# python-microscopy/ch-shrinkwrap

Measured on AMD Instinct MI355X. Metric: vertex-updates/s (force+CG step) + achieved HBM GB/s, 1M pts/200k verts, higher is better.
Workload: dtype f32; 1 GPU; BASELINE configs[2]: two-lobe vesicle (smooth union of two R=300 nm spheres), 1000000 localizations sigma=10 nm, 198812 vertices / 397620 faces, lams=[10], blocks of 5 iterations, fixed topology; localizations_per_gpu=1000000, vertices_per_gpu=198812, faces_per_gpu=397620, block=5, mode=single, parallelism=single GPU

## Files before the change

ch_shrinkwrap_amd/build.py:

```python
import glob
import os
import subprocess

HERE = os.path.dirname(os.path.abspath(__file__))
LIB = os.path.join(HERE, 'libnanowrap_hip.so')


def _csrc(name):
    return os.path.join(HERE, 'csrc', name)


def _include(name):
    return os.path.join(os.path.dirname(HERE), 'include', name)


HIPCC_FLAGS = ['-O3', '--offload-arch=gfx950', '-fPIC', '-shared', '-ffp-contract=off', '-munsafe-fp-atomics',
               '-fvisibility=hidden', '-Wall', '-Wno-unused-function']
_BASE = ['-O3', '--offload-arch=gfx950', '-fPIC', '-fvisibility=hidden']
_QUERY = _BASE + ['-ffp-contract=off', '-Wall', '-Wno-unused-function']
_BQ_H = [_csrc('nw_bq.h'), _csrc('nw_bq_core.h')]
_BQ = _BQ_H + [_csrc('nw_device.h')]

OBJ_MAIN, OBJ_HOLEPUNCH, OBJ_SURGERY, OBJ_BQ = _csrc('nanowrap.o'), _csrc('nw_holepunch.o'), _csrc('nw_surgery.o'), _csrc('nw_bq.o')
OBJ_ISOSURFACE = _csrc('nw_isosurface.o')
# ... 50 lines not shown
        if verbose:
            print(' '.join(cmd))
        subprocess.check_call(cmd)

    for src, obj, extra, flags in UNITS:
        if force or not os.path.exists(obj) or os.path.getmtime(obj) < max(os.path.getmtime(d) for d in [src] + extra):
            run([hipcc] + flags + ['-c', '-o', obj, src])
    check_kernel_budgets(verbose=verbose)
    run([hipcc, '--offload-arch=gfx950', '-fPIC', '-shared', '-o', LIB] + [obj for _, obj, _, _ in UNITS])
    return LIB


LLVM_BIN = os.environ.get('NW_LLVM_BIN', '/opt/rocm/lib/llvm/bin')
KERNEL_BUDGETS = {
    'k_nn_wave<false>':               (80, 10 * 1024),
    'k_attract':                      (72, 20 * 1024),
    'k_face_centroids':               (64, 8 * 1024),
    'k_centroid_scatter':             (64, 0),
    'k_scan_final':                   (64, 1024),
    'k_prior_ring':                   (128, 1024),
    'k_prior_directions':             (96, 1024),
    'k_subspace_point_sums':          (128, 1024),
    'k_solve_update':                 (128, 1024),
    'k_hp_empty_faces':               (64, 0),
    'k_hp_pair':                      (64, 8 * 1024),
    'k_hp_prism':                     (176, 0),
    'k_hp_cand_geom':                 (32, 0),
    'k_hp_pair_final':                (16, 0),
    'k_ws_init':                      (16, 0),
    'k_ws_hook':                      (32, 0),
    'k_ws_compress':                  (16, 0),
    'k_ws_number':                    (16, 0),
    'k_ws_stats':                     (64, 0),
    'k_ws_bbox_init':                 (16, 0),
    'k_ws_active':                    (16, 0),
    'k_ws_winding':                   (176, 0),
    'k_ws_lengths':                   (16, 0),
    'k_ws_hist':                      (16, 2048),
    'k_ws_pick':                      (32, 0),
    'k_ws_flag':                      (16, 0),
    'k_iso_count':                    (16, 16 * 1024),
    'k_iso_widen':                    (16, 0),
    'k_iso_smooth':                   (16, 0),
    'k_iso_hist':                     (16, 1024),
    'k_iso_pattern':                  (32, 0),
    'k_iso_compact':                  (16, 0),
# ... 152 lines not shown
```

ch_shrinkwrap_amd/csrc/nanowrap.hip:

```cpp
#include <hip/hip_runtime.h>
#include <cstdio>
#include <cstdlib>
#include <cstring>
#include <cmath>
#include <string>
#include <vector>
#include <algorithm>
#include <chrono>
#include <thread>
#include <atomic>

#include "../../include/nanowrap.h"
#include "nw_kernels.h"
#include "nw_host_copy.h"

int nw_sort_pairs_u32(const unsigned *key_in, unsigned *key_out, const int *val_in, int *val_out, int n, int bits, hipStream_t stream);

static_assert(sizeof(NwIterLogDev) == sizeof(nw_iter_log), "device/host log record mismatch");
static_assert(SC_COUNT <= NW_N_SCALARS, "scalar slots");

#define NW_EXPORT extern "C" __attribute__((visibility("default")))

#include <dlfcn.h>
#include <rccl/rccl.h>
struct NwRccl {
    void *lib = nullptr;
    ncclResult_t (*GetUniqueId)(ncclUniqueId *) = nullptr;
    ncclResult_t (*CommInitRank)(ncclComm_t *, int, ncclUniqueId, int) = nullptr;
    ncclResult_t (*CommDestroy)(ncclComm_t) = nullptr;
    ncclResult_t (*AllReduce)(const void *, void *, size_t, ncclDataType_t, ncclRedOp_t, ncclComm_t, hipStream_t) = nullptr;
    ncclResult_t (*Send)(const void *, size_t, ncclDataType_t, int, ncclComm_t, hipStream_t) = nullptr;
    ncclResult_t (*Recv)(void *, size_t, ncclDataType_t, int, ncclComm_t, hipStream_t) = nullptr;
    ncclResult_t (*GroupStart)() = nullptr;
    ncclResult_t (*GroupEnd)() = nullptr;
    const char *(*GetErrorString)(ncclResult_t) = nullptr;
    std::string err;
// ... 99 lines not shown
    double cell_tune = 1.0;
    bool tuned = false;
    int blocks_done = 0;
    double force_h = 0.0;
    DevBuf<int> ccount, cstart, scan_tmp;
    DevBuf<int> ctile;
    DevBuf<float> data_in, dat;
    bool have_data = false;
    DevBuf<NwItem> items;
    DevBuf<unsigned> item_cost;
    bool handoff_off = false;
    DevBuf<int> query_serial;
    DevBuf<int> item_done;
    bool items_by_cost = false;
    bool item_cost_valid = false;
    int nitems = 0;
    int item_level = -1;
    DevBuf<int> aux_i;
    DevBuf<float> aux_f, aux_f2, aux_f3;
    DevBuf<double> aux_d;
    DevBuf<unsigned long long> nn_stats;
    DevBuf<unsigned> proj_key;
    DevBuf<int> proj_idx;
    bool proj_ready = false, proj_sorted = false;
    bool face_warm = false;

    DevBuf<float> pos, meshpos, nrm;
    DevBuf<int> nbr, nbr_t, faces;
    DevBuf<unsigned char> valid, owned;
    bool have_valid = false, have_owned = false;
    DevBuf<int> hb_local, hb_slot, hb_slot2local, hb_gv;
    DevBuf<long long> halo_acc;
    DevBuf<float> halo_rows;
    DevBuf<float> halo_full;
    DevBuf<float> halo_ref;
    DevBuf<float> halo_d0;
    bool have_halo_d0 = false;
    int64_t halo_d0_n = 0;
    DevBuf<float> halo_stats;
    void *pin_full = nullptr;
    size_t pin_full_bytes = 0;
    bool full_staged = false;
    bool have_halo_ref = false;
    int64_t hb_n = 0, hb_nslot = 0, M_global = 0;
    bool have_boundary = false;
    bool pos_unpack_pending = false;
    bool have_peers = false;
// ... 146 lines not shown
    const double sr = ctx->sigma_eff > 0 ? std::min(std::max(ctx->sigma_eff / sp, 1.0), 16.0) : 4.0;
    double h = 2.9 * sp * std::pow(sr, 0.3) * std::pow(ratio, -0.11);
    const char *e = getenv("NW_CELL_FACTOR");
    if (e && atof(e) > 0) h *= atof(e);
    return std::max(h, 0.5 * mean_dist) * ctx->cell_tune;
}

int ensure_item_done(nw_ctx *ctx)
{
    const size_t want = (size_t)std::max(ctx->nitems, 1) + 256;
    if (!ctx->query_serial.p) {
        NW_HIP(ctx->query_serial.ensure(1));
        NW_HIP(hipMemsetAsync(ctx->query_serial.p, 0, sizeof(int), ctx->stream));
    }
    if (ctx->item_done.n < want) {
        NW_HIP(ctx->item_done.ensure(2 * want));
        NW_HIP(hipMemsetAsync(ctx->item_done.p, 0, 2 * want * sizeof(int), ctx->stream));
    }
    const size_t rows = (size_t)(ctx->nitems + 8 * 16 + 8);
    if (ctx->part_a.n < 5 * rows) NW_HIP(ctx->part_a.ensure(5 * rows));
    return NW_OK;
}

int build_items(nw_ctx *ctx, int level)
{
    const int64_t N = ctx->N;
    int ipts = (N >= 64 * 9216) ? NW_ITEM_POINTS : NW_ITEM_POINTS / 2;
    if (const char *e = getenv("NW_ITEM_PTS")) ipts = std::max(8, std::min(NW_ITEM_POINTS, atoi(e)));
    if (level == ctx->item_level && ctx->nitems > 0 && ipts == ctx->item_points) return NW_OK;
    ctx->item_points = ipts;
    DevBuf<int> head, hscan, bstart, icount, istart;
    NW_HIP(head.ensure(N)); NW_HIP(hscan.ensure(N + 1));
    hipLaunchKernelGGL(k_block_heads, dim3(nblk(N)), dim3(NW_BLOCK), 0, ctx->stream, ctx->mkey.p, (int)N, 3 * level, head.p);
    NW_TRY(scan_exclusive(ctx, head.p, (int)N, hscan.p));
    int nblocks = 0;
    NW_HIP(hipMemcpyAsync(&nblocks, hscan.p + N, sizeof(int), hipMemcpyDeviceToHost, ctx->stream));
    NW_HIP(hipStreamSynchronize(ctx->stream));
    NW_HIP(bstart.ensure((size_t)nblocks + 1)); NW_HIP(icount.ensure((size_t)nblocks)); NW_HIP(istart.ensure((size_t)nblocks + 1));
    hipLaunchKernelGGL(k_block_starts, dim3(nblk(N)), dim3(NW_BLOCK), 0, ctx->stream, head.p, hscan.p, (int)N, bstart.p);
    hipLaunchKernelGGL(k_block_item_counts, dim3(nblk(nblocks)), dim3(NW_BLOCK), 0, ctx->stream, bstart.p, nblocks, icount.p, ctx->item_points);
    NW_TRY(scan_exclusive(ctx, icount.p, nblocks, istart.p));
    int nitems = 0;
    NW_HIP(hipMemcpyAsync(&nitems, istart.p + nblocks, sizeof(int), hipMemcpyDeviceToHost, ctx->stream));
    NW_HIP(hipStreamSynchronize(ctx->stream));
    NW_HIP(ctx->items.ensure((size_t)nitems));
    hipLaunchKernelGGL(k_block_fill_items, dim3(nblk(nblocks)), dim3(NW_BLOCK), 0, ctx->stream, bstart.p, istart.p, nblocks, ctx->items.p, ctx->item_points);
    NW_HIP(hipGetLastError());
    NW_HIP(hipStreamSynchronize(ctx->stream));
    ctx->nitems = nitems;
    ctx->item_level = level;
    NW_HIP(ctx->item_cost.ensure((size_t)2 * nitems));
    NW_HIP(hipMemsetAsync(ctx->item_cost.p, 0, (size_t)2 * nitems * sizeof(unsigned), ctx->stream));
    NW_TRY(ensure_item_done(ctx));
    ctx->items_by_cost = false; ctx->item_cost_valid = false;
    if (getenv("NW_VERBOSE"))
        fprintf(stderr, "[nanowrap] work list: Morton level %d (block %.2f), %d blocks, %d items (%.1f localizations per wave)\n", level,
                ctx->morton_unit * (float)(1 << level), nblocks, nitems, (double)N / std::max(nitems, 1));
    return NW_OK;
}

int build_grid(nw_ctx *ctx, double mean_dist)
{
    const int64_t N = ctx->N, F = ctx->F;
    float mlo[3], mhi[3];
    bool bad = false;
    NW_TRY(minmax3(ctx, ctx->meshpos.p, ctx->M, mlo, mhi, &bad));
    if (bad) return fail(ctx, NW_ERR_NONFINITE, "non-finite vertex coordinate");
    NW_HIP(ctx->wsum.ensure(4));
    NW_HIP(hipMemsetAsync(ctx->wsum.p + 1, 0, 2 * sizeof(double), ctx->stream));
    hipLaunchKernelGGL(k_mesh_area, dim3(std::min(1024, nblk(F))), dim3(NW_BLOCK), 0, ctx->stream, ctx->meshpos.p, ctx->faces.p, (int)F, ctx->wsum.p + 1);
    const int nsample = (int)std::min<int64_t>(N, 256);
    if (mean_dist <= 0.0)
        hipLaunchKernelGGL(k_sample_nn, dim3(nsample), dim3(NW_BLOCK), 0, ctx->stream, ctx->pts_in.p, N, nsample, ctx->meshpos.p, ctx->faces.p, (int)F, ctx->wsum.p + 2);
    NW_HIP(hipGetLastError());
    double h2[2];
    NW_HIP(hipMemcpyAsync(h2, ctx->wsum.p + 1, sizeof(h2), hipMemcpyDeviceToHost, ctx->stream));
    NW_HIP(hipStreamSynchronize(ctx->stream));
// ... 316 lines not shown
                           1.0f / ctx->morton_unit, key_in.p, idx_in.p);
        NW_HIP(hipGetLastError());
        const int se = nw_sort_pairs_u32(key_in.p, ctx->mkey.p, idx_in.p, ctx->perm.p, (int)N, 30, ctx->stream);
        if (se != 0) return fail(ctx, NW_ERR_HIP, std::string("radix sort of the Morton keys: ") + hipGetErrorString((hipError_t)se));
        NW_HIP(ctx->pts.ensure(N));
        NW_HIP(ctx->mask.ensure(N));
        if (ctx->sinv_array) NW_HIP(ctx->sinv.ensure(3 * N));
        if (ctx->w_array) NW_HIP(ctx->wnorm.ensure(3 * N));
        const float *w_src = ctx->w_array ? ((ctx->w_mode == NW_WEIGHTS_ARRAY || ctx->w_mode == NW_WEIGHTS_PRENORMALIZED) ? ctx->w_in.p : ctx->sinv_in.p) : nullptr;
        hipLaunchKernelGGL(k_point_gather, dim3(nblk(N)), dim3(NW_BLOCK), 0, ctx->stream, (int)N, ctx->pts_in.p, ctx->perm.p,
                           ctx->sinv_array ? ctx->sinv_in.p : nullptr, w_src, ctx->wsum.p, ctx->w_array ? (ctx->w_mode == NW_WEIGHTS_PRENORMALIZED ? 2 : 1) : 0,
                           ctx->pts.p, ctx->sinv_array ? ctx->sinv.p : nullptr, ctx->w_array ? ctx->wnorm.p : nullptr, ctx->mask.p);
        NW_HIP(hipGetLastError());
        NW_HIP(hipStreamSynchronize(ctx->stream));
    }
    ctx->have_points = true;
    ctx->have_data = false;
    ctx->grid_valid = false;
    ctx->item_level = -1;
    ctx->nitems = 0;
    ctx->face_warm = false;
    if (verbose_level() >= 2) fprintf(stderr, "[nanowrap] warm start dropped (%s)\n", __func__);
    ctx->proj_ready = false; ctx->proj_sorted = false;
    ctx->tuned = false; ctx->cell_tune = 1.0; ctx->blocks_done = 0;
    ctx->last_mean_dist = -1.0;
    ctx->searched = false;
    return NW_OK;
}

static int gather_data(nw_ctx *ctx)
{
    const int64_t N = ctx->N;
    if (ctx->have_data) NW_HIP(ctx->dat.ensure(3 * N));
    hipLaunchKernelGGL(k_data_gather, dim3(nblk(N)), dim3(NW_BLOCK), 0, ctx->stream, (int)N, ctx->perm.p, ctx->have_data ? ctx->data_in.p : nullptr, ctx->pts.p,
                       ctx->have_data ? ctx->dat.p : nullptr, ctx->w_array ? nullptr : ctx->mask.p);
    NW_HIP(hipGetLastError());
    return NW_OK;
}

NW_EXPORT int nw_set_data(nw_ctx *ctx, const float *data)
{
    if (!ctx) return NW_ERR_BADARG;
    if (!ctx->have_points) return fail(ctx, NW_ERR_BADARG, "nw_set_data: set the localizations first");
    if (ctx->in_search) return fail(ctx, NW_ERR_BADARG, "nw_set_data inside a search");
    NW_HIP(hipSetDevice(ctx->device));
    if (!data && !ctx->have_data) return NW_OK;
// ... 337 lines not shown
        for (int k = 0; k < 3; ++k) ext = std::max(ext, (double)mhi[k] - (double)mlo[k]);
    }
    const double q = std::ldexp(1.0, (int)std::ceil(std::log2(ext * ext)) - 44);
    hipLaunchKernelGGL(k_normals_scatter, dim3(nblk(ctx->F)), dim3(NW_BLOCK), 0, ctx->stream, (int)ctx->F, ctx->faces.p, ctx->meshpos.p, ctx->vacc.p, 1.0 / q);
    hipLaunchKernelGGL(k_normals_finish, dim3(nblk(ctx->M)), dim3(NW_BLOCK), 0, ctx->stream, (int)ctx->M, ctx->vacc.p, ctx->nrm.p);
    NW_HIP(hipGetLastError());
    if (nrm_out) NW_HIP(hipMemcpyAsync(nrm_out, ctx->nrm.p, 3 * ctx->M * sizeof(float), hipMemcpyDefault, ctx->stream));
    NW_HIP(hipStreamSynchronize(ctx->stream));
    return NW_OK;
}

NW_EXPORT int nw_reset_history(nw_ctx *ctx)
{
    if (!ctx || !ctx->have_mesh) return fail(ctx, NW_ERR_BADARG, "nw_reset_history: mesh not set");
    if (ctx->in_search) return fail(ctx, NW_ERR_BADARG, "nw_reset_history inside a search");
    NwDevState st{};
    st.stop_at = 0x7fffffff;
    NW_HIP(hipMemcpyAsync(ctx->state.p, &st, sizeof(st), hipMemcpyHostToDevice, ctx->stream));
    NW_HIP(hipStreamSynchronize(ctx->stream));
    ctx->global_iter = 0;
    return NW_OK;
}

static int resort_by_projection(nw_ctx *ctx)
{
    const int64_t N = ctx->N;
    DevBuf<int> order;
    DevBuf<float4> pts2;
    DevBuf<int> perm2, face2;
    DevBuf<float> sinv2, wnorm2;
    DevBuf<unsigned char> mask2;
    NW_HIP(order.ensure(N)); NW_HIP(pts2.ensure(N)); NW_HIP(perm2.ensure(N)); NW_HIP(face2.ensure(N)); NW_HIP(mask2.ensure(N));
    if (ctx->sinv_array) NW_HIP(sinv2.ensure(3 * N));
    if (ctx->w_array) NW_HIP(wnorm2.ensure(3 * N));
    const int se = nw_sort_pairs_u32(ctx->proj_key.p, ctx->mkey.p, ctx->proj_idx.p, order.p, (int)N, 30, ctx->stream);
    if (se != 0) return fail(ctx, NW_ERR_HIP, std::string("radix sort of the projection keys: ") + hipGetErrorString((hipError_t)se));
    hipLaunchKernelGGL(k_point_regather, dim3(nblk(N)), dim3(NW_BLOCK), 0, ctx->stream, (int)N, order.p, ctx->pts.p, ctx->perm.p,
                       ctx->sinv_array ? ctx->sinv.p : nullptr, ctx->w_array ? ctx->wnorm.p : nullptr, ctx->mask.p, ctx->face.p,
                       pts2.p, perm2.p, sinv2.p, wnorm2.p, mask2.p, face2.p);
    NW_HIP(hipGetLastError());
    NW_HIP(hipStreamSynchronize(ctx->stream));
    ctx->pts.swap(pts2); ctx->perm.swap(perm2); ctx->mask.swap(mask2); ctx->face.swap(face2);
    if (ctx->sinv_array) ctx->sinv.swap(sinv2);
    if (ctx->w_array) ctx->wnorm.swap(wnorm2);
    ctx->morton_unit = ctx->proj_unit;
    ctx->item_level = -1; ctx->nitems = 0;
    ctx->grid_valid = false;
    ctx->proj_sorted = true; ctx->proj_ready = false;
    ctx->searched = false;
    ctx->proj_key.release(); ctx->proj_idx.release();
    if (ctx->have_data) NW_TRY(gather_data(ctx));
    if (getenv("NW_VERBOSE")) fprintf(stderr, "[nanowrap] localizations re-sorted by their foot point on the surface\n");
    return NW_OK;
}

enum { QP_GRID = 1, QP_NN = 2, QP_FIXUP = 4, QP_ATTRACT = 8, QP_ALL = 15 };
static int launch_query(nw_ctx *ctx, int it, int parts = QP_GRID | QP_NN | QP_FIXUP, bool with_ring = false, bool with_attract = false, bool *attract_rode = nullptr);
static NwAttractArgs attract_args(const nw_ctx *ctx);
static nw_ctx::BlockGraph *block_graph(nw_ctx *ctx, int num_iters, bool head = false);
static int tune_grid(nw_ctx *ctx)
{
    if (ctx->tuned) return NW_OK;
    const bool autotune = env_on("NW_AUTOTUNE");
    if (!autotune || getenv("NW_CELL_SIZE") || getenv("NW_CELL_FACTOR") || ctx->N < 20000 || !ctx->face_warm) {
        if (ctx->face_warm || !autotune) ctx->tuned = true;
        return NW_OK;
    }
    ctx->tuned = true;
    const int verbose = getenv("NW_VERBOSE") != nullptr;
    const int it = 0;
    hipLaunchKernelGGL(k_set_iter_base, dim3(1), dim3(1), 0, ctx->stream, ctx->state.p, ctx->global_iter);
    const int prof = ctx->profiling;
    ctx->profiling = 0;
// ... 472 lines not shown
                fprintf(stderr, "[nanowrap] search_end: wait + sliced write-back %ld us\n", (long)std::chrono::duration_cast<std::chrono::microseconds>(std::chrono::steady_clock::now() - tw0).count());
        }
    }
    const auto ts0 = std::chrono::steady_clock::now();
    ctx->direct_out = false;
    ctx->done_launched = false; ctx->sliced_S = 0;
    NW_HIP(hipStreamSynchronize(ctx->stream));
    if (verbose_level() >= 3)
        fprintf(stderr, "[nanowrap] search_end: final synchronize %ld us\n", (long)std::chrono::duration_cast<std::chrono::microseconds>(std::chrono::steady_clock::now() - ts0).count());
    const NwDevState st = *stp;
    int executed = 0;
    for (int i = 0; i < ctx->search_done; ++i) executed += host[i].executed ? 1 : 0;
    if (loopcount) *loopcount = executed;
    if (log) for (int i = 0; i < ctx->search_done; ++i) log[i] = host[i];
    if (executed > 0) ctx->last_mean_dist = host[executed - 1].mean_dist;
    ctx->searched = ctx->searched || executed > 0;
    if (executed > 0) ctx->blocks_done += 1;
    if (st.grid_escape) ctx->grid_valid = false;
    if (executed > 0 && !ctx->proj_sorted && !ctx->proj_ready && ctx->face_warm) {
        const NwGrid &g = ctx->grid;
        const double ext = std::max({(double)g.gx, (double)g.gy, (double)g.gz}) * g.h;
        ctx->proj_unit = (float)(ext / 1024.0);
        NW_HIP(ctx->proj_key.ensure(ctx->N)); NW_HIP(ctx->proj_idx.ensure(ctx->N));
        hipLaunchKernelGGL(k_projection_keys, dim3(nblk(ctx->N)), dim3(NW_BLOCK), 0, ctx->stream, (int)ctx->N, ctx->face.p, (int)ctx->F, ctx->cent_tmp.p, ctx->pts.p,
                           g.ox, g.oy, g.oz, 1.0f / ctx->proj_unit, ctx->proj_key.p, ctx->proj_idx.p);
        NW_HIP(hipGetLastError());
        NW_HIP(hipStreamSynchronize(ctx->stream));
        ctx->proj_ready = true;
    }
    if (ctx->profiling) {
        for (auto &sp : g_marks.spans) {
            float ms = 0;
            if (hipEventElapsedTime(&ms, sp.second.first, sp.second.second) == hipSuccess) { ctx->stage_ms[sp.first] += ms; ctx->stage_ms[ST_TOTAL] += ms; }
        }
        g_marks.spans.clear();
    }
    if (st.status != 0) {
        const int code = st.status;
        NwDevState st2 = st; st2.status = 0;
        st2.stop_at = 0x7fffffff;
        (void)hipMemcpy(ctx->state.p, &st2, sizeof(st2), hipMemcpyHostToDevice);
        if (code == NW_ERR_NAN) return fail(ctx, NW_ERR_NAN, "NaN detected in weight matrix / A f / A^T r (reference asserts at mesh_conj_grad.py:514,548,580)");
        if (code == NW_ERR_SINGULAR) return fail(ctx, NW_ERR_SINGULAR, "singular subspace normal equations (numpy.linalg.solve would raise LinAlgError)");
        if (code == NW_ERR_INTERNAL) return fail(ctx, NW_ERR_INTERNAL, "internal error: the nearest-face query produced an invalid face id");
        if (code == NW_ERR_HANDOFF) {
            ctx->handoff_off = true;
            for (auto &gph : ctx->graphs) if (gph.exec) { (void)hipGraphExecDestroy(gph.exec); gph.exec = nullptr; }
            return fail(ctx, NW_ERR_HANDOFF, "the attraction step inside the query launch gave up waiting for its work item (200 ms); the ctx now runs the two as separate launches: run the block again");
// ... 667 lines not shown
    NW_HIP(hipMemset(ctx->nn_stats.p, 0, h.size() * sizeof(unsigned long long)));
    for (int k = 0; k < NWS_COUNT; ++k) {
        unsigned long long v = 0;
        for (int c = 0; c < NWS_COPIES; ++c) v = (k == NWS_T_WAVE_MAX) ? std::max(v, h[(size_t)c * NWS_COUNT + k]) : v + h[(size_t)c * NWS_COUNT + k];
        out[k] = (int64_t)v;
    }
    out[NWS_COUNT] = ctx->nitems;
    return NW_OK;
}

NW_EXPORT int nw_debug(nw_ctx *ctx, int what, void *a, void *b, int cap, int *n)
{
    if (what == 0) return debug_nn_stats(ctx, (int64_t *)a);
    if (what == 1) return debug_items(ctx, (int32_t *)a, (uint32_t *)b, cap, n);
    if (what == 2 && ctx && a) {
        ((int64_t *)a)[0] = ctx->n_staged_copy_outs; ((int64_t *)a)[1] = ctx->n_write_backs;
        return NW_OK;
    }
    if (what == 3 && ctx) {
        if (ctx->in_search) return fail(ctx, NW_ERR_BADARG, "nw_debug(3) inside a search");
        ctx->handoff_off = cap != 0;
        return NW_OK;
    }
    return NW_ERR_BADARG;
}

NW_EXPORT int nw_accumulator_quantum(nw_ctx *ctx, double *q)
{
    if (!ctx || !q) return NW_ERR_BADARG;
    if (*q != 0 && ctx->in_search && ctx->search_done > 0) return fail(ctx, NW_ERR_BADARG, "nw_accumulator_quantum: cannot change the quantum between the iterations of a search");
    if (*q > 0 && std::isfinite(*q)) {
        int e = 0;
        const double m = std::frexp(*q, &e);
        ctx->quantum_override = std::ldexp(1.0, m == 0.5 ? e - 1 : e);
        if (ctx->in_search) ctx->acc_quantum = ctx->quantum_override;
    } else if (*q < 0) {
        ctx->quantum_override = 0.0;
        if (ctx->in_search) ctx->acc_quantum = ctx->local_quantum;
    }
    if (!ctx->in_search && ctx->have_points && ctx->have_mesh) {
        NW_HIP(hipSetDevice(ctx->device));
        NW_TRY(alloc_work(ctx));
        NW_TRY(ensure_grid(ctx));
        ctx->local_quantum = std::ldexp(1.0, (int)std::ceil(std::log2(std::max(ctx->scene_ext * ctx->w_bound, 1e-300))) - 36);
    }
    *q = ctx->local_quantum;
// ... 19 lines not shown
```

ch_shrinkwrap_amd/csrc/nw_nn.h:

```cpp
#pragma once
#include "nw_device.h"

#define NW_NN_TOL 6e-6f
#define NW_NN_TOLK 4e-6f
#define NW_NN_CULL 4e-6f
#define NW_ITEM_POINTS 64
#define NW_OUTLIERS 8
#define NW_NNA_HT 256
#define NW_NNA_HT_BITS 8

struct NwItem { int p0, n; };

__device__ __forceinline__ unsigned nw_spread10(unsigned v)
{
    v &= 0x3ffu;
    v = (v | (v << 16)) & 0x030000ffu;
    v = (v | (v << 8)) & 0x0300f00fu;
    v = (v | (v << 4)) & 0x030c30c3u;
    v = (v | (v << 2)) & 0x09249249u;
    return v;
}

__global__ void k_morton_keys(const float *__restrict__ xyz, int N, float lox, float loy, float loz, float inv_unit, unsigned *__restrict__ key, int *__restrict__ idx)
{
// ... 54 lines not shown
{
    const int slot = blockIdx.x * blockDim.x + threadIdx.x;
    if (slot >= N) return;
    const int i = order[slot];
    const float x = xyz[3 * i], y = xyz[3 * i + 1], z = xyz[3 * i + 2];
    pts[slot] = make_float4(x, y, z, __int_as_float(i));
    if (sinv_in)
        for (int k = 0; k < 3; ++k) sinv[3 * slot + k] = sinv_in[3 * i + k];
    unsigned m = 0;
    if (w_is_array) {
        const float mean = (float)(wsum[0] / (3.0 * (double)N));
        for (int k = 0; k < 3; ++k) {
            const float w = w_in[3 * i + k];
            wnorm[3 * slot + k] = (w_is_array == 2) ? w : w / mean;
            m |= (w > 0.0f) ? (1u << k) : 0u;
        }
    } else {
        m = (isfinite(x) ? 1u : 0u) | (isfinite(y) ? 2u : 0u) | (isfinite(z) ? 4u : 0u);
    }
    mask[slot] = (unsigned char)m;
}

__global__ void k_projection_keys(int N, const int *__restrict__ face, int F, const float4 *__restrict__ cent_by_face, const float4 *__restrict__ pts,
                                  float lox, float loy, float loz, float inv_unit, unsigned *__restrict__ key, int *__restrict__ idx)
{
    const int i = blockIdx.x * blockDim.x + threadIdx.x;
    if (i >= N) return;
    const int f = face[i];
    const float4 C = ((unsigned)f < (unsigned)F) ? cent_by_face[f] : pts[i];
    const int qx = nw_clampi((int)((C.x - lox) * inv_unit), 0, 1023);
    const int qy = nw_clampi((int)((C.y - loy) * inv_unit), 0, 1023);
    const int qz = nw_clampi((int)((C.z - loz) * inv_unit), 0, 1023);
    key[i] = nw_spread10((unsigned)qx) | (nw_spread10((unsigned)qy) << 1) | (nw_spread10((unsigned)qz) << 2);
    idx[i] = i;
}

__global__ void k_point_regather(int N, const int *__restrict__ order, const float4 *__restrict__ pts_o, const int *__restrict__ perm_o,
                                 const float *__restrict__ sinv_o, const float *__restrict__ wnorm_o, const unsigned char *__restrict__ mask_o, const int *__restrict__ face_o,
                                 float4 *__restrict__ pts, int *__restrict__ perm, float *__restrict__ sinv, float *__restrict__ wnorm, unsigned char *__restrict__ mask,
                                 int *__restrict__ face)
{
    const int s = blockIdx.x * blockDim.x + threadIdx.x;
    if (s >= N) return;
    const int o = order[s];
    pts[s] = pts_o[o];
    perm[s] = perm_o[o];
    mask[s] = mask_o[o];
    face[s] = face_o[o];
    if (sinv_o)
        for (int k = 0; k < 3; ++k) sinv[3 * s + k] = sinv_o[3 * o + k];
    if (wnorm_o)
        for (int k = 0; k < 3; ++k) wnorm[3 * s + k] = wnorm_o[3 * o + k];
// ... 574 lines not shown
```

Before: 761.3 million vertex-updates/s.

## Partition localizations into k-d leaves by surface foot point for work items

After the projection-key radix sort, each Morton block is recursively split with a GPU k-d partition over the foot point and a weighted height coordinate. Within each leaf, points are then ordered by face. The leaves become the nearest-neighbour work items in place of Morton-block chunking, aiming for tighter spatial groups per wave and better locality in the per-iteration force and search kernels. The cost is several extra kernels and host syncs during the resort, which runs once at setup and not in the per-iteration loop. It also adds a large-LDS partition kernel and new debug paths.

```diff
diff --git a/ch_shrinkwrap_amd/build.py b/ch_shrinkwrap_amd/build.py
--- a/ch_shrinkwrap_amd/build.py
+++ b/ch_shrinkwrap_amd/build.py
@@ -96,6 +96,12 @@
     'k_prior_directions':             (96, 1024),
     'k_subspace_point_sums':          (128, 1024),
     'k_solve_update':                 (128, 1024),
+    'k_kd_block_max':                 (16, 0),
+    'k_kd_seg_counts':                (16, 0),
+    'k_kd_fill_segs':                 (32, 0),
+    'k_kd_leaf_counts':               (16, 0),
+    'k_kd_fill_leaves':               (32, 0),
+    'k_kd_partition':                 (64, 146 * 1024),
     'k_hp_empty_faces':               (64, 0),
     'k_hp_pair':                      (64, 8 * 1024),
     'k_hp_prism':                     (176, 0),
diff --git a/ch_shrinkwrap_amd/csrc/nanowrap.hip b/ch_shrinkwrap_amd/csrc/nanowrap.hip
--- a/ch_shrinkwrap_amd/csrc/nanowrap.hip
+++ b/ch_shrinkwrap_amd/csrc/nanowrap.hip
@@ -12,6 +12,7 @@
 
 #include "../../include/nanowrap.h"
 #include "nw_kernels.h"
+#include "nw_partition.h"
 #include "nw_host_copy.h"
 
 int nw_sort_pairs_u32(const unsigned *key_in, unsigned *key_out, const int *val_in, int *val_out, int n, int bits, hipStream_t stream);
@@ -157,7 +158,13 @@
     DevBuf<unsigned long long> nn_stats;
     DevBuf<unsigned> proj_key;
     DevBuf<int> proj_idx;
+    DevBuf<float4> proj_foot;
     bool proj_ready = false, proj_sorted = false;
+    DevBuf<NwItem> kd_leaves;
+    int kd_nleaves = 0, kd_leaf = 0, kd_nsegs = 0, kd_level = 0;
+    std::vector<uint32_t> kd_dbg_key;
+    std::vector<float> kd_dbg_foot;
+    std::vector<int> kd_dbg_face, kd_dbg_perm;
     bool face_warm = false;
 
     DevBuf<float> pos, meshpos, nrm;
@@ -350,11 +357,39 @@
     return NW_OK;
 }
 
+static int wanted_item_points(const nw_ctx *ctx)
+{
+    int ipts = (ctx->N >= 64 * 9216) ? NW_ITEM_POINTS : NW_ITEM_POINTS / 2;
+    if (const char *e = getenv("NW_ITEM_PTS")) ipts = std::max(8, std::min(NW_ITEM_POINTS, atoi(e)));
+    return ipts;
+}
+
+static int finish_items(nw_ctx *ctx, int nitems, int level)
+{
+    ctx->nitems = nitems;
+    ctx->item_level = level;
+    NW_HIP(ctx->item_cost.ensure((size_t)2 * nitems));
+    NW_HIP(hipMemsetAsync(ctx->item_cost.p, 0, (size_t)2 * nitems * sizeof(unsigned), ctx->stream));
+    NW_TRY(ensure_item_done(ctx));
+    ctx->items_by_cost = false; ctx->item_cost_valid = false;
+    return NW_OK;
+}
+
 int build_items(nw_ctx *ctx, int level)
 {
     const int64_t N = ctx->N;
-    int ipts = (N >= 64 * 9216) ? NW_ITEM_POINTS : NW_ITEM_POINTS / 2;
-    if (const char *e = getenv("NW_ITEM_PTS")) ipts = std::max(8, std::min(NW_ITEM_POINTS, atoi(e)));
+    const int ipts = wanted_item_points(ctx);
+    if (ctx->kd_nleaves > 0 && ipts == ctx->kd_leaf) {
+        if (ctx->nitems > 0 && ctx->item_level >= 0 && ipts == ctx->item_points) { ctx->item_level = level; return NW_OK; }
+        ctx->item_points = ipts;
+        NW_HIP(ctx->items.ensure((size_t)ctx->kd_nleaves));
+        NW_HIP(hipMemcpyAsync(ctx->items.p, ctx->kd_leaves.p, (size_t)ctx->kd_nleaves * sizeof(NwItem), hipMemcpyDeviceToDevice, ctx->stream));
+        NW_TRY(finish_items(ctx, ctx->kd_nleaves, level));
+        if (getenv("NW_VERBOSE"))
+            fprintf(stderr, "[nanowrap] work list: k-d leaves of %d start segments (Morton level %d), %d items (%.1f localizations per wave)\n", ctx->kd_nsegs,
+                    ctx->kd_level, ctx->nitems, (double)N / std::max(ctx->nitems, 1));
+        return NW_OK;
+    }
     if (level == ctx->item_level && ctx->nitems > 0 && ipts == ctx->item_points) return NW_OK;
     ctx->item_points = ipts;
     DevBuf<int> head, hscan, bstart, icount, istart;
@@ -375,12 +410,7 @@
     hipLaunchKernelGGL(k_block_fill_items, dim3(nblk(nblocks)), dim3(NW_BLOCK), 0, ctx->stream, bstart.p, istart.p, nblocks, ctx->items.p, ctx->item_points);
     NW_HIP(hipGetLastError());
     NW_HIP(hipStreamSynchronize(ctx->stream));
-    ctx->nitems = nitems;
-    ctx->item_level = level;
-    NW_HIP(ctx->item_cost.ensure((size_t)2 * nitems));
-    NW_HIP(hipMemsetAsync(ctx->item_cost.p, 0, (size_t)2 * nitems * sizeof(unsigned), ctx->stream));
-    NW_TRY(ensure_item_done(ctx));
-    ctx->items_by_cost = false; ctx->item_cost_valid = false;
+    NW_TRY(finish_items(ctx, nitems, level));
     if (getenv("NW_VERBOSE"))
         fprintf(stderr, "[nanowrap] work list: Morton level %d (block %.2f), %d blocks, %d items (%.1f localizations per wave)\n", level,
                 ctx->morton_unit * (float)(1 << level), nblocks, nitems, (double)N / std::max(nitems, 1));
@@ -743,6 +773,7 @@
     ctx->face_warm = false;
     if (verbose_level() >= 2) fprintf(stderr, "[nanowrap] warm start dropped (%s)\n", __func__);
     ctx->proj_ready = false; ctx->proj_sorted = false;
+    ctx->kd_nleaves = 0;
     ctx->tuned = false; ctx->cell_tune = 1.0; ctx->blocks_done = 0;
     ctx->last_mean_dist = -1.0;
     ctx->searched = false;
@@ -1126,6 +1157,84 @@
     return NW_OK;
 }
 
+static bool kd_sort_on()
+{
+    static const bool on = [] { const char *e = getenv("NW_KD_SORT"); return e ? atoi(e) != 0 : true; }();
+    return on;
+}
+static float kd_height_weight()
+{
+    static const float w = [] { const char *e = getenv("NW_KD_HEIGHT"); return e ? (float)atof(e) : 0.5f; }();
+    return w;
+}
+
+static int kd_partition(nw_ctx *ctx, DevBuf<int> &order)
+{
+    const int N = (int)ctx->N;
+    const int leaf = wanted_item_points(ctx);
+    ctx->kd_nleaves = 0;
+    if (N < 1 || leaf < NWP_MIN_LEAF || leaf % 4 != 0 || !ctx->proj_foot.p) return NW_OK;
+    const int cap = NWP_CAP / leaf * leaf;
+    const float w = kd_height_weight();
+    const auto t0 = std::chrono::steady_clock::now();
+    DevBuf<int> maxb, head, hscan, bstart, cnt, cscan, lcnt, lscan, order2;
+    DevBuf<NwItem> segs;
+    int hmax[nwp::LEVELS];
+    NW_HIP(maxb.ensure(nwp::LEVELS));
+    NW_HIP(hipMemsetAsync(maxb.p, 0, sizeof(hmax), ctx->stream));
+    hipLaunchKernelGGL(k_kd_block_max, dim3(nblk(N)), dim3(NW_BLOCK), 0, ctx->stream, ctx->mkey.p, N, maxb.p);
+    NW_HIP(hipMemcpyAsync(hmax, maxb.p, sizeof(hmax), hipMemcpyDeviceToHost, ctx->stream));
+    NW_HIP(hipStreamSynchronize(ctx->stream));
+    const int level = nwp::start_level(hmax, cap);
+    NW_HIP(head.ensure(N)); NW_HIP(hscan.ensure((size_t)N + 1));
+    hipLaunchKernelGGL(k_block_heads, dim3(nblk(N)), dim3(NW_BLOCK), 0, ctx->stream, ctx->mkey.p, N, 3 * level, head.p);
+    NW_TRY(scan_exclusive(ctx, head.p, N, hscan.p));
+    int nblocks = 0, nsegs = 0, nleaves = 0;
+    NW_HIP(hipMemcpyAsync(&nblocks, hscan.p + N, sizeof(int), hipMemcpyDeviceToHost, ctx->stream));
+    NW_HIP(hipStreamSynchronize(ctx->stream));
+    NW_HIP(bstart.ensure((size_t)nblocks + 1));
+    hipLaunchKernelGGL(k_block_starts, dim3(nblk(N)), dim3(NW_BLOCK), 0, ctx->stream, head.p, hscan.p, N, bstart.p);
+    NW_HIP(cnt.ensure((size_t)nblocks)); NW_HIP(cscan.ensure((size_t)nblocks + 1));
+    hipLaunchKernelGGL(k_kd_seg_counts, dim3(nblk(nblocks)), dim3(NW_BLOCK), 0, ctx->stream, bstart.p, nblocks, cap, leaf, cnt.p);
+    NW_TRY(scan_exclusive(ctx, cnt.p, nblocks, cscan.p));
+    NW_HIP(hipMemcpyAsync(&nsegs, cscan.p + nblocks, sizeof(int), hipMemcpyDeviceToHost, ctx->stream));
+    NW_HIP(hipStreamSynchronize(ctx->stream));
+    NW_HIP(segs.ensure((size_t)nsegs));
+    hipLaunchKernelGGL(k_kd_fill_segs, dim3(nblk(nblocks)), dim3(NW_BLOCK), 0, ctx->stream, bstart.p, cscan.p, nblocks, cap, leaf, segs.p);
+    NW_HIP(lcnt.ensure((size_t)nsegs)); NW_HIP(lscan.ensure((size_t)nsegs + 1));
+    hipLaunchKernelGGL(k_kd_leaf_counts, dim3(nblk(nsegs)), dim3(NW_BLOCK), 0, ctx->stream, segs.p, nsegs, leaf, lcnt.p);
+    NW_TRY(scan_exclusive(ctx, lcnt.p, nsegs, lscan.p));
+    NW_HIP(hipMemcpyAsync(&nleaves, lscan.p + nsegs, sizeof(int), hipMemcpyDeviceToHost, ctx->stream));
+    NW_HIP(hipStreamSynchronize(ctx->stream));
+    NW_HIP(ctx->kd_leaves.ensure((size_t)nleaves));
+    hipLaunchKernelGGL(k_kd_fill_leaves, dim3(nblk(nsegs)), dim3(NW_BLOCK), 0, ctx->stream, segs.p, lscan.p, nsegs, leaf, ctx->kd_leaves.p);
+    NW_HIP(order2.ensure(N));
+    hipLaunchKernelGGL(k_kd_partition, dim3(nsegs), dim3(NWP_THREADS), 0, ctx->stream, segs.p, nsegs, order.p, ctx->proj_foot.p, ctx->face.p, leaf, w, order2.p);
+    NW_HIP(hipGetLastError());
+    NW_HIP(hipStreamSynchronize(ctx->stream));
+    if (getenv("NW_KD_KEEP")) {
+        std::vector<int> ord(N), face(N), perm(N);
+        std::vector<float> foot(4 * (size_t)N);
+        ctx->kd_dbg_key.resize(N); ctx->kd_dbg_foot.resize(4 * (size_t)N); ctx->kd_dbg_face.resize(N); ctx->kd_dbg_perm.resize(N);
+        NW_HIP(hipMemcpy(ord.data(), order.p, (size_t)N * sizeof(int), hipMemcpyDeviceToHost));
+        NW_HIP(hipMemcpy(face.data(), ctx->face.p, (size_t)N * sizeof(int), hipMemcpyDeviceToHost));
+        NW_HIP(hipMemcpy(perm.data(), ctx->perm.p, (size_t)N * sizeof(int), hipMemcpyDeviceToHost));
+        NW_HIP(hipMemcpy(foot.data(), ctx->proj_foot.p, 4 * (size_t)N * sizeof(float), hipMemcpyDeviceToHost));
+        NW_HIP(hipMemcpy(ctx->kd_dbg_key.data(), ctx->mkey.p, (size_t)N * sizeof(uint32_t), hipMemcpyDeviceToHost));
+        for (int s = 0; s < N; ++s) {
+            const int o = ord[s];
+            ctx->kd_dbg_face[s] = face[o]; ctx->kd_dbg_perm[s] = perm[o];
+            for (int k = 0; k < 4; ++k) ctx->kd_dbg_foot[4 * (size_t)s + k] = foot[4 * (size_t)o + k];
+        }
+    }
+    if (getenv("NW_VERBOSE"))
+        fprintf(stderr, "[nanowrap] k-d partition: %d start segments at Morton level %d (largest block %d), %d leaves of %d, height weight %.2f: %ld us\n", nsegs, level,
+                hmax[level], nleaves, leaf, w, (long)std::chrono::duration_cast<std::chrono::microseconds>(std::chrono::steady_clock::now() - t0).count());
+    order.swap(order2);
+    ctx->kd_nleaves = nleaves; ctx->kd_leaf = leaf; ctx->kd_nsegs = nsegs; ctx->kd_level = level;
+    return NW_OK;
+}
+
 static int resort_by_projection(nw_ctx *ctx)
 {
     const int64_t N = ctx->N;
@@ -1139,6 +1248,7 @@
     if (ctx->w_array) NW_HIP(wnorm2.ensure(3 * N));
     const int se = nw_sort_pairs_u32(ctx->proj_key.p, ctx->mkey.p, ctx->proj_idx.p, order.p, (int)N, 30, ctx->stream);
     if (se != 0) return fail(ctx, NW_ERR_HIP, std::string("radix sort of the projection keys: ") + hipGetErrorString((hipError_t)se));
+    if (kd_sort_on()) NW_TRY(kd_partition(ctx, order));
     hipLaunchKernelGGL(k_point_regather, dim3(nblk(N)), dim3(NW_BLOCK), 0, ctx->stream, (int)N, order.p, ctx->pts.p, ctx->perm.p,
                        ctx->sinv_array ? ctx->sinv.p : nullptr, ctx->w_array ? ctx->wnorm.p : nullptr, ctx->mask.p, ctx->face.p,
                        pts2.p, perm2.p, sinv2.p, wnorm2.p, mask2.p, face2.p);
@@ -1152,7 +1262,7 @@
     ctx->grid_valid = false;
     ctx->proj_sorted = true; ctx->proj_ready = false;
     ctx->searched = false;
-    ctx->proj_key.release(); ctx->proj_idx.release();
+    ctx->proj_key.release(); ctx->proj_idx.release(); ctx->proj_foot.release();
     if (ctx->have_data) NW_TRY(gather_data(ctx));
     if (getenv("NW_VERBOSE")) fprintf(stderr, "[nanowrap] localizations re-sorted by their foot point on the surface\n");
     return NW_OK;
@@ -1671,8 +1781,10 @@
         const double ext = std::max({(double)g.gx, (double)g.gy, (double)g.gz}) * g.h;
         ctx->proj_unit = (float)(ext / 1024.0);
         NW_HIP(ctx->proj_key.ensure(ctx->N)); NW_HIP(ctx->proj_idx.ensure(ctx->N));
+        const bool kd = kd_sort_on() && !getenv("NW_NO_PROJ_SORT");
+        if (kd) NW_HIP(ctx->proj_foot.ensure(ctx->N));
         hipLaunchKernelGGL(k_projection_keys, dim3(nblk(ctx->N)), dim3(NW_BLOCK), 0, ctx->stream, (int)ctx->N, ctx->face.p, (int)ctx->F, ctx->cent_tmp.p, ctx->pts.p,
-                           g.ox, g.oy, g.oz, 1.0f / ctx->proj_unit, ctx->proj_key.p, ctx->proj_idx.p);
+                           g.ox, g.oy, g.oz, 1.0f / ctx->proj_unit, ctx->proj_key.p, ctx->proj_idx.p, ctx->pos.p, ctx->faces.p, kd ? ctx->proj_foot.p : (float4 *)nullptr);
         NW_HIP(hipGetLastError());
         NW_HIP(hipStreamSynchronize(ctx->stream));
         ctx->proj_ready = true;
@@ -2386,6 +2498,25 @@
         ctx->handoff_off = cap != 0;
         return NW_OK;
     }
+    if (what == 4 && ctx && a && n) {
+        *n = (int)ctx->N;
+        if (b) {
+            int32_t *kd = (int32_t *)b;
+            const float w = kd_height_weight();
+            kd[0] = ctx->kd_nleaves; kd[1] = ctx->kd_nleaves > 0 ? ctx->kd_nsegs : 0; kd[2] = ctx->kd_nleaves > 0 ? ctx->kd_level : 0;
+            kd[3] = ctx->kd_nleaves > 0 ? ctx->kd_leaf : 0;
+            memcpy(&kd[4], &w, 4);
+        }
+        if (ctx->perm.p && cap > 0) NW_HIP(hipMemcpy(a, ctx->perm.p, (size_t)std::min<int64_t>(cap, ctx->N) * sizeof(int), hipMemcpyDeviceToHost));
+        return NW_OK;
+    }
+    if ((what == 5 || what == 6) && ctx && a && b && n) {
+        const size_t have = ctx->kd_dbg_key.size(), m = std::min<size_t>((size_t)std::max(cap, 0), have);
+        *n = (int)have;
+        if (what == 5) { memcpy(a, ctx->kd_dbg_key.data(), m * sizeof(uint32_t)); memcpy(b, ctx->kd_dbg_foot.data(), 4 * m * sizeof(float)); }
+        else { memcpy(a, ctx->kd_dbg_face.data(), m * sizeof(int)); memcpy(b, ctx->kd_dbg_perm.data(), m * sizeof(int)); }
+        return NW_OK;
+    }
     return NW_ERR_BADARG;
 }
 
diff --git a/ch_shrinkwrap_amd/csrc/nw_nn.h b/ch_shrinkwrap_amd/csrc/nw_nn.h
--- a/ch_shrinkwrap_amd/csrc/nw_nn.h
+++ b/ch_shrinkwrap_amd/csrc/nw_nn.h
@@ -100,12 +100,27 @@
 }
 
 __global__ void k_projection_keys(int N, const int *__restrict__ face, int F, const float4 *__restrict__ cent_by_face, const float4 *__restrict__ pts,
-                                  float lox, float loy, float loz, float inv_unit, unsigned *__restrict__ key, int *__restrict__ idx)
+                                  float lox, float loy, float loz, float inv_unit, unsigned *__restrict__ key, int *__restrict__ idx,
+                                  const float *__restrict__ pos, const int *__restrict__ faces, float4 *__restrict__ foot)
 {
     const int i = blockIdx.x * blockDim.x + threadIdx.x;
     if (i >= N) return;
     const int f = face[i];
     const float4 C = ((unsigned)f < (unsigned)F) ? cent_by_face[f] : pts[i];
+    if (foot) {
+        float h = 0.0f;
+        if ((unsigned)f < (unsigned)F) {
+            const int a = faces[3 * f], b = faces[3 * f + 1], c = faces[3 * f + 2];
+            const float ax = pos[3 * a], ay = pos[3 * a + 1], az = pos[3 * a + 2];
+            const float ux = pos[3 * b] - ax, uy = pos[3 * b + 1] - ay, uz = pos[3 * b + 2] - az;
+            const float vx = pos[3 * c] - ax, vy = pos[3 * c + 1] - ay, vz = pos[3 * c + 2] - az;
+            const float nx = uy * vz - uz * vy, ny = uz * vx - ux * vz, nz = ux * vy - uy * vx;
+            const float4 P = pts[i];
+            h = ((P.x - C.x) * nx + (P.y - C.y) * ny + (P.z - C.z) * nz) * rsqrtf(nx * nx + ny * ny + nz * nz);
+            if (!isfinite(h)) h = 0.0f;
+        }
+        foot[i] = make_float4(C.x, C.y, C.z, h);
+    }
     const int qx = nw_clampi((int)((C.x - lox) * inv_unit), 0, 1023);
     const int qy = nw_clampi((int)((C.y - loy) * inv_unit), 0, 1023);
     const int qz = nw_clampi((int)((C.z - loz) * inv_unit), 0, 1023);
diff --git a/ch_shrinkwrap_amd/csrc/nw_partition.h b/ch_shrinkwrap_amd/csrc/nw_partition.h
--- /dev/null
+++ b/ch_shrinkwrap_amd/csrc/nw_partition.h
@@ -0,0 +1,206 @@
+#pragma once
+#include "nw_partition_core.h"
+
+#define NWP_CAP 16384
+#define NWP_MIN_LEAF 32
+#define NWP_THREADS 1024
+
+__global__ void k_kd_block_max(const unsigned *__restrict__ key, int N, int *__restrict__ max_block)
+{
+    const int i = blockIdx.x * blockDim.x + threadIdx.x;
+    if (i >= N) return;
+    const unsigned k = key[i];
+    for (int l = 0; l < nwp::LEVELS; ++l) {
+        const int shift = 3 * l;
+        if (i > 0 && (key[i - 1] >> shift) == (k >> shift)) break;
+        int lo = i + 1, hi = N;
+        while (lo < hi) {
+            const int mid = lo + ((hi - lo) >> 1);
+            if ((key[mid] >> shift) == (k >> shift)) lo = mid + 1; else hi = mid;
+        }
+        if (lo - i > __atomic_load_n(&max_block[l], __ATOMIC_RELAXED)) atomicMax(&max_block[l], lo - i);
+    }
+}
+
+__global__ void k_kd_seg_counts(const int *__restrict__ bstart, int nblocks, int cap, int leaf, int *__restrict__ nsegs)
+{
+    const int b = blockIdx.x * blockDim.x + threadIdx.x;
+    if (b >= nblocks) return;
+    nsegs[b] = nwp::chunk_count(bstart[b + 1] - bstart[b], cap, leaf);
+}
+
+__global__ void k_kd_fill_segs(const int *__restrict__ bstart, const int *__restrict__ sstart, int nblocks, int cap, int leaf, NwItem *__restrict__ segs)
+{
+    const int b = blockIdx.x * blockDim.x + threadIdx.x;
+    if (b >= nblocks) return;
+    const int p0 = bstart[b], p1 = bstart[b + 1], m = p1 - p0;
+    if (m <= 0) return;
+    const int per = m > cap ? nwp::chunk_len(m, cap, leaf) : m;
+    int o = sstart[b];
+    for (int p = p0; p < p1; p += per) {
+        NwItem s;
+        s.p0 = p; s.n = min(per, p1 - p);
+        segs[o++] = s;
+    }
+}
+
+__global__ void k_kd_leaf_counts(const NwItem *__restrict__ segs, int nsegs, int leaf, int *__restrict__ nleaves)
+{
+    const int s = blockIdx.x * blockDim.x + threadIdx.x;
+    if (s >= nsegs) return;
+    nleaves[s] = (segs[s].n + leaf - 1) / leaf;
+}
+
+__global__ void k_kd_fill_leaves(const NwItem *__restrict__ segs, const int *__restrict__ lstart, int nsegs, int leaf, NwItem *__restrict__ leaves)
+{
+    const int s = blockIdx.x * blockDim.x + threadIdx.x;
+    if (s >= nsegs) return;
+    const NwItem sg = segs[s];
+    int o = lstart[s];
+    for (int p = 0; p < sg.n; p += leaf) {
+        NwItem w;
+        w.p0 = sg.p0 + p; w.n = min(leaf, sg.n - p);
+        leaves[o++] = w;
+    }
+}
+
+__device__ __forceinline__ int nwkd_rank_u32(const unsigned *comp, int s0, int n, unsigned me)
+{
+    const uint4 *c4 = reinterpret_cast<const uint4 *>(comp + s0);
+    int rank = 0;
+    const int q = n >> 2;
+    for (int t = 0; t < q; ++t) {
+        const uint4 v = c4[t];
+        rank += (v.x < me ? 1 : 0) + (v.y < me ? 1 : 0) + (v.z < me ? 1 : 0) + (v.w < me ? 1 : 0);
+    }
+    for (int t = s0 + 4 * q; t < s0 + n; ++t) rank += comp[t] < me ? 1 : 0;
+    return rank;
+}
+
+__device__ __forceinline__ void nwkd_part_segment(const unsigned short *idx_in, unsigned short *idx_out, const unsigned *keys, int s0, int n, int nl,
+                                                 unsigned *hist, int *wsum, int *pick)
+{
+    const int tid = (int)threadIdx.x, lane = tid & 63, wave = tid >> 6;
+    int below = 0;
+    unsigned prefix = 0;
+    for (int pass = 0; pass < 2; ++pass) {
+        const int shift = pass == 0 ? 8 : 0;
+        if (tid < 256) hist[tid] = 0u;
+        __syncthreads();
+        for (int j = s0 + tid; j < s0 + n; j += NWP_THREADS) {
+            const unsigned k = keys[j];
+            if (pass == 0 || (k >> 8) == prefix) atomicAdd(&hist[(k >> shift) & 255u], 1u);
+        }
+        __syncthreads();
+        if (tid == 0) {
+            int acc = below, b = 0;
+            while (b < 255 && acc + (int)hist[b] < nl) { acc += (int)hist[b]; ++b; }
+            pick[0] = b; pick[1] = acc;
+        }
+        __syncthreads();
+        prefix = (prefix << 8) | (unsigned)pick[0];
+        below = pick[1];
+        __syncthreads();
+    }
+    const unsigned K = prefix;
+    const int take = nl - below;
+    const int per = (n + NWP_THREADS - 1) / NWP_THREADS;
+    const int j0 = min(s0 + tid * per, s0 + n), j1 = min(j0 + per, s0 + n);
+    int lt = 0, eq = 0;
+    for (int j = j0; j < j1; ++j) { const unsigned k = keys[j]; lt += k < K ? 1 : 0; eq += k == K ? 1 : 0; }
+    const int lt_in = nw_wave_incl_scan(lt, lane), eq_in = nw_wave_incl_scan(eq, lane);
+    if (lane == 63) { wsum[wave] = lt_in; wsum[16 + wave] = eq_in; }
+    __syncthreads();
+    int lt_before = lt_in - lt, eq_before = eq_in - eq;
+    for (int v = 0; v < wave; ++v) { lt_before += wsum[v]; eq_before += wsum[16 + v]; }
+    int left_before = lt_before + min(eq_before, take);
+    for (int j = j0; j < j1; ++j) {
+        const unsigned k = keys[j];
+        const bool left = k < K || (k == K && eq_before < take);
+        eq_before += k == K ? 1 : 0;
+        const int to = left ? s0 + left_before : s0 + nl + (j - s0 - left_before);
+        left_before += left ? 1 : 0;
+        idx_out[to] = idx_in[j];
+    }
+    __syncthreads();
+}
+
+__global__ __launch_bounds__(NWP_THREADS) void k_kd_partition(const NwItem *__restrict__ segs, int nsegs, const int *__restrict__ order_in,
+                                                              const float4 *__restrict__ foot, const int *__restrict__ face, int leaf, float w,
+                                                              int *__restrict__ order_out)
+{
+    __shared__ unsigned short idx[2][NWP_CAP];
+    __shared__ __attribute__((aligned(16))) unsigned comp[NWP_CAP];
+    __shared__ unsigned box[NWP_CAP / NWP_MIN_LEAF][2 * nwp::AXES];
+    __shared__ unsigned hist[256];
+    __shared__ int wsum[2 * (NWP_THREADS / 64)], pick[4];
+    if ((int)blockIdx.x >= nsegs) return;
+    const NwItem sg = segs[blockIdx.x];
+    const int n = sg.n, p0 = sg.p0, tid = (int)threadIdx.x;
+    if (n > NWP_CAP || leaf < NWP_MIN_LEAF) {
+        for (int j = tid; j < n; j += NWP_THREADS) order_out[p0 + j] = order_in[p0 + j];
+        return;
+    }
+    for (int j = tid; j < n; j += NWP_THREADS) idx[0][j] = (unsigned short)j;
+    int cur = 0;
+    for (int depth = 0; depth < nwp::MAX_DEPTH; ++depth) {
+        int any = 0;
+        for (int j = tid; j < n; j += NWP_THREADS) any |= nwp::seg_at(n, leaf, depth, j).n > leaf ? 1 : 0;
+        for (int k = tid; k < (NWP_CAP / NWP_MIN_LEAF) * 2 * nwp::AXES; k += NWP_THREADS)
+            box[k / (2 * nwp::AXES)][k % (2 * nwp::AXES)] = (k % (2 * nwp::AXES)) < nwp::AXES ? 0xffffffffu : 0u;
+        if (!__syncthreads_or(any)) break;
+        for (int j = tid; j < n; j += NWP_THREADS) {
+            const nwp::Seg s = nwp::seg_at(n, leaf, depth, j);
+            if (s.n <= leaf) continue;
+            const float4 f = foot[order_in[p0 + idx[cur][j]]];
+            float c[nwp::AXES];
+            nwp::coords(f.x, f.y, f.z, f.w, w, c);
+            unsigned *b = box[s.s0 / leaf];
+            for (int a = 0; a < nwp::AXES; ++a) {
+                const unsigned e = nwp::enc(c[a]);
+                atomicMin(&b[a], e);
+                atomicMax(&b[nwp::AXES + a], e);
+            }
+        }
+        __syncthreads();
+        for (int j = tid; j < n; j += NWP_THREADS) {
+            const nwp::Seg s = nwp::seg_at(n, leaf, depth, j);
+            if (s.n <= leaf) continue;
+            const unsigned *b = box[s.s0 / leaf];
+            float lo[nwp::AXES], hi[nwp::AXES];
+            for (int a = 0; a < nwp::AXES; ++a) { lo[a] = nwp::dec(b[a]); hi[a] = nwp::dec(b[nwp::AXES + a]); }
+            const int axis = nwp::widest_axis(lo, hi);
+            const float4 f = foot[order_in[p0 + idx[cur][j]]];
+            float c[nwp::AXES];
+            nwp::coords(f.x, f.y, f.z, f.w, w, c);
+            const float v = axis == 0 ? c[0] : axis == 1 ? c[1] : axis == 2 ? c[2] : c[3];
+            const float vlo = axis == 0 ? lo[0] : axis == 1 ? lo[1] : axis == 2 ? lo[2] : lo[3];
+            const float vhi = axis == 0 ? hi[0] : axis == 1 ? hi[1] : axis == 2 ? hi[2] : hi[3];
+            const unsigned key = nwp::quantise(v, vlo, vhi);
+            comp[j] = s.n > nwp::SORT_MAX ? key : (key << 16) | (unsigned)j;
+        }
+        __syncthreads();
+        for (int j = 0; j < n;) {
+            const nwp::Seg s = nwp::seg_at(n, leaf, depth, j);
+            j = s.s0 + s.n;
+            if (s.n > nwp::SORT_MAX) nwkd_part_segment(idx[cur], idx[cur ^ 1], comp, s.s0, s.n, nwp::cut_rank(s.n, leaf), hist, wsum, pick);
+        }
+        for (int j = tid; j < n; j += NWP_THREADS) {
+            const nwp::Seg s = nwp::seg_at(n, leaf, depth, j);
+            if (s.n > nwp::SORT_MAX) continue;
+            const int to = s.n > leaf ? s.s0 + nwkd_rank_u32(comp, s.s0, s.n, comp[j]) : j;
+            idx[cur ^ 1][to] = idx[cur][j];
+        }
+        cur ^= 1;
+        __syncthreads();
+    }
+    for (int j = tid; j < n; j += NWP_THREADS) comp[j] = (unsigned)face[order_in[p0 + idx[cur][j]]];
+    __syncthreads();
+    for (int j = tid; j < n; j += NWP_THREADS) {
+        const int l0 = j / leaf * leaf, l1 = min(l0 + leaf, n);
+        const int fj = (int)comp[j];
+        int rank = 0;
+        for (int t = l0; t < l1; ++t) rank += nwp::face_before((int)comp[t], t, fj, j) ? 1 : 0;
+        order_out[p0 + l0 + rank] = order_in[p0 + idx[cur][j]];
+    }
+}
diff --git a/ch_shrinkwrap_amd/csrc/nw_partition_core.h b/ch_shrinkwrap_amd/csrc/nw_partition_core.h
--- /dev/null
+++ b/ch_shrinkwrap_amd/csrc/nw_partition_core.h
@@ -0,0 +1,182 @@
+#pragma once
+#include <cstdint>
+#include <cstring>
+
+#if defined(__HIPCC__)
+#define NWP_HD __host__ __device__ __forceinline__
+#else
+#define NWP_HD inline
+#endif
+
+namespace nwp {
+
+enum { AXES = 4, LEVELS = 11, MAX_DEPTH = 32, SORT_MAX = 1024 };
+
+NWP_HD float clean(float v) { return (v - v == 0.0f) ? v + 0.0f : 0.0f; }
+
+NWP_HD uint32_t enc(float f)
+{
+    uint32_t b;
+    memcpy(&b, &f, 4);
+    return (b & 0x80000000u) ? ~b : (b | 0x80000000u);
+}
+NWP_HD float dec(uint32_t e)
+{
+    const uint32_t b = (e & 0x80000000u) ? (e & 0x7fffffffu) : ~e;
+    float f;
+    memcpy(&f, &b, 4);
+    return f;
+}
+
+NWP_HD void coords(float fx, float fy, float fz, float height, float w, float c[AXES])
+{
+    c[0] = clean(fx); c[1] = clean(fy); c[2] = clean(fz); c[3] = clean(w * clean(height));
+}
+
+NWP_HD int cut_rank(int n, int leaf) { return ((n + leaf - 1) / leaf / 2) * leaf; }
+
+struct Seg { int s0, n; };
+NWP_HD Seg seg_at(int n, int leaf, int depth, int j)
+{
+    Seg s;
+    s.s0 = 0; s.n = n;
+    for (int d = 0; d < depth && s.n > leaf; ++d) {
+        const int nl = cut_rank(s.n, leaf);
+        if (j < s.s0 + nl) s.n = nl;
+        else { s.s0 += nl; s.n -= nl; }
+    }
+    return s;
+}
+
+NWP_HD int widest_axis(const float lo[AXES], const float hi[AXES])
+{
+    int best = 0;
+    float e = hi[0] - lo[0];
+    for (int a = 1; a < AXES; ++a) {
+        const float ea = hi[a] - lo[a];
+        if (ea > e) { e = ea; best = a; }
+    }
+    return best;
+}
+
+NWP_HD uint32_t quantise(float v, float lo, float hi)
+{
+    const float ext = hi - lo;
+    if (!(ext > 0.0f)) return 0u;
+    const float scale = 65535.0f / ext;
+    if (!(scale - scale == 0.0f)) return 0u;
+    const float x = (v - lo) * scale;
+    if (!(x < 65535.0f)) return 65535u;
+    return x > 0.0f ? (uint32_t)x : 0u;
+}
+
+NWP_HD bool face_before(int fa, int ja, int fb, int jb) { return fa < fb || (fa == fb && ja < jb); }
+
+NWP_HD int start_level(const int max_block[LEVELS], int cap)
+{
+    for (int l = LEVELS - 1; l > 0; --l)
+        if (max_block[l] <= cap) return l;
+    return 0;
+}
+
+NWP_HD int chunk_len(int m, int cap, int leaf)
+{
+    const int k = (m + cap - 1) / cap;
+    const int per = (m + k - 1) / k;
+    return (per + leaf - 1) / leaf * leaf;
+}
+NWP_HD int chunk_count(int m, int cap, int leaf)
+{
+    if (m <= cap) return 1;
+    const int per = chunk_len(m, cap, leaf);
+    return (m + per - 1) / per;
+}
+
+}
+
+#if !defined(__HIP_DEVICE_COMPILE__)
+#include <algorithm>
+#include <vector>
+
+namespace nwp {
+
+struct HostResult {
+    std::vector<int> order;
+    std::vector<int> seg_start;
+    std::vector<int> leaf_start;
+    int level = 0;
+};
+
+inline HostResult partition_host(int n, const uint32_t *key, const float *foot, const int *face, int leaf, int cap, float w, int sort_max = SORT_MAX)
+{
+    HostResult r;
+    int max_block[LEVELS];
+    for (int l = 0; l < LEVELS; ++l) {
+        max_block[l] = 0;
+        for (int i = 0, b0 = 0; i <= n; ++i)
+            if (i == n || (i > 0 && (key[i] >> (3 * l)) != (key[i - 1] >> (3 * l)))) { max_block[l] = std::max(max_block[l], i - b0); b0 = i; }
+    }
+    r.level = start_level(max_block, cap);
+    const int shift = 3 * r.level;
+    for (int i = 0, b0 = 0; i <= n; ++i)
+        if (i == n || (i > 0 && (key[i] >> shift) != (key[i - 1] >> shift))) {
+            const int m = i - b0, per = m > cap ? chunk_len(m, cap, leaf) : m;
+            for (int p = b0; p < i; p += per) r.seg_start.push_back(p);
+            b0 = i;
+        }
+    r.seg_start.push_back(n);
+    r.order.resize((size_t)n);
+    for (int i = 0; i < n; ++i) r.order[(size_t)i] = i;
+    std::vector<uint32_t> k16((size_t)n);
+    for (size_t s = 0; s + 1 < r.seg_start.size(); ++s) {
+        const int p0 = r.seg_start[s], m = r.seg_start[s + 1] - p0;
+        int *ord = r.order.data() + p0;
+        bool more = true;
+        for (int depth = 0; more && depth < MAX_DEPTH; ++depth) {
+            more = false;
+            for (int j = 0; j < m;) {
+                const Seg sg = seg_at(m, leaf, depth, j);
+                j = sg.s0 + sg.n;
+                if (sg.n <= leaf) continue;
+                more = true;
+                uint32_t lo[AXES], hi[AXES];
+                for (int a = 0; a < AXES; ++a) { lo[a] = 0xffffffffu; hi[a] = 0u; }
+                float c[AXES];
+                for (int t = sg.s0; t < sg.s0 + sg.n; ++t) {
+                    const float *f = foot + 4 * (size_t)ord[t];
+                    coords(f[0], f[1], f[2], f[3], w, c);
+                    for (int a = 0; a < AXES; ++a) { lo[a] = std::min(lo[a], enc(c[a])); hi[a] = std::max(hi[a], enc(c[a])); }
+                }
+                float flo[AXES], fhi[AXES];
+                for (int a = 0; a < AXES; ++a) { flo[a] = dec(lo[a]); fhi[a] = dec(hi[a]); }
+                const int axis = widest_axis(flo, fhi);
+                for (int t = sg.s0; t < sg.s0 + sg.n; ++t) {
+                    const float *f = foot + 4 * (size_t)ord[t];
+                    coords(f[0], f[1], f[2], f[3], w, c);
+                    k16[(size_t)ord[t]] = quantise(c[axis], flo[axis], fhi[axis]);
+                }
+                int *b = ord + sg.s0, *e = b + sg.n;
+                if (sg.n <= sort_max) {
+                    std::stable_sort(b, e, [&](int x, int y) { return k16[(size_t)x] < k16[(size_t)y]; });
+                } else {
+                    std::vector<int> by_key(b, e);
+                    std::stable_sort(by_key.begin(), by_key.end(), [&](int x, int y) { return k16[(size_t)x] < k16[(size_t)y]; });
+                    const int nl = cut_rank(sg.n, leaf);
+                    std::vector<char> left((size_t)n, 0);
+                    for (int t = 0; t < nl; ++t) left[(size_t)by_key[(size_t)t]] = 1;
+                    std::stable_partition(b, e, [&](int x) { return left[(size_t)x] != 0; });
+                }
+            }
+        }
+        for (int j = 0; j < m; j += leaf) {
+            const int len = std::min(leaf, m - j);
+            r.leaf_start.push_back(p0 + j);
+            std::stable_sort(ord + j, ord + j + len, [&](int x, int y) { return face[x] < face[y]; });
+        }
+    }
+    r.leaf_start.push_back(n);
+    return r;
+}
+
+}
+#endif
```

After: 821.2 million vertex-updates/s, median of 6. +7.9%, better.
